# caidj0/Raytracer-2025

Hardware: NVIDIA B200
Metric: paths_per_sec (higher is better)
Workload: dtype f64

## Files before the change

raytracer-2025_b200/csrc/api.cu:

```cuda
#include <cuda_runtime.h>

#include <algorithm>
#include <cstdio>
#include <cstdlib>
#include <cstring>
#include <memory>
#include <mutex>
#include <new>
#include <string>
#include <thread>
#include <vector>

#include "compile.h"
#include "kernels.h"
#include "rt2025.h"

using namespace rt;

namespace {

thread_local std::string g_err;

int set_err(int code, const std::string& msg) {
    g_err = msg;
// ... 326 lines not shown
            v.nodes = a.put(cs.nodes, st), v.geom = a.put(cs.geom, st), v.meta = a.put(cs.meta, st), v.xforms = a.put(cs.xforms, st);
            v.materials = a.put(cs.materials, st), v.textures = a.put(cs.textures, st), v.images = a.put(cs.images, st);
            v.texels = a.put(cs.texels, st), v.perlins = a.put(cs.perlins, st), v.media = a.put(cs.media, st);
            v.lights = a.put(cs.lights, st), v.remaps = a.put(cs.remaps, st), v.walk_lean = a.put(cs.walk_lean, st);
            v.shade_lean = a.put(cs.shade_lean, st), v.shade_lean_mask = cs.shade_lean_mask;
            CU(cudaStreamSynchronize(st));
        }
        v.world_root = cs.world_root;
        v.n_media = (uint32_t)cs.media.size();
        v.n_xforms = (uint32_t)cs.xforms.size();
        v.kinds = (cs.n_spheres && !cs.n_planars) ? 1u : ((cs.n_planars && !cs.n_spheres) ? 2u : 0u);
        v.n_lights = (uint32_t)cs.lights.size();
        v.n_prims = (uint32_t)cs.geom.size();
        v.moving = 0;
        for (size_t p = 0; p < cs.geom.size(); p++)
            if ((cs.meta[p].kind_mat >> 30) == PRIM_SPHERE && (cs.geom[p].d[3] != 0.0 || cs.geom[p].d[4] != 0.0 || cs.geom[p].d[5] != 0.0)) v.moving = 1;
        s->ranks = cs.ranks;
        for (auto& m : cs.media) s->generic_media |= m.single_sphere == RT_NONE;
        v.media_xform = 0;
        for (auto& m : cs.media)
            if (m.xform != RT_NONE || (m.single_sphere != RT_NONE && cs.meta[m.single_sphere].xform != RT_NONE)) v.media_xform = 1;
        for (auto& m : cs.materials) s->class_mask |= 1u << m.shade_class;
        for (auto& t : cs.textures) s->black_texture.push_back(t.kind == RT_TEX_SOLID && t.color[0] == 0.0 && t.color[1] == 0.0 && t.color[2] == 0.0);
        uint32_t n_thick = 0, n_thick_entries = 0;
        for (auto& m : cs.media)
            if (m.flags & MEDIUM_THICK) s->class_mask |= 1u << SC_WALK, n_thick++, n_thick_entries += m.n_entry != MEDIUM_NO_ENTRIES;
        v.walk_entries_only = n_thick == 1 && n_thick_entries == 1;
        s->lights_flat = 1;
        for (auto& l : cs.lights)
            if (l.weight != 1.0 / (double)cs.lights.size()) s->lights_flat = 0;
        rt_scene_info& i = s->info;
// ... 776 lines not shown
```

raytracer-2025_b200/csrc/compile.cpp:

```cpp
#include "compile.h"

#include <omp.h>

#include <memory>
#include <parallel/algorithm>

#include <chrono>
#include <cstdio>
#include <cstdlib>

#include <vector_functions.h>

#include <algorithm>
#include <cmath>
#include <cstring>
#include <limits>

namespace rt {

namespace {

struct V3 {
    double x, y, z;
};
// ... 318 lines not shown
        double inv[9];
        if (!out_chain.inverse(inv)) return fail(RT_ERR_UNSUPPORTED, "singular Transform (zero scale)");
        return true;
    }

    bool leaf(uint32_t obj, const Affine& a, PrimGeom& g, uint32_t& kind, double lo[3], double hi[3], double* area_out, bool quiet = false) {
        const rt_object& o = d.objects[obj];
        std::memset(&g, 0, sizeof(g));
        V3 pts[8];
        int np = 0;
        double pad_r = 0.0;
        if (o.kind == RT_OBJ_SPHERE) {
            const rt_sphere& s = d.spheres[o.data];
            V3 c = v3(s.center), cv = v3(s.center_vec);
            double r = s.radius;
            g.d[0] = c.x, g.d[1] = c.y, g.d[2] = c.z, g.d[3] = cv.x, g.d[4] = cv.y, g.d[5] = cv.z, g.d[6] = r;
            kind = PRIM_SPHERE;
            if (area_out) *area_out = 0.0;
            V3 c1 = c + cv;
            bool similarity = true;
            double k = 1.0;
            if (!a.identity) {
                k = a.A[0] * a.A[0] + a.A[3] * a.A[3] + a.A[6] * a.A[6];
                for (int i = 0; i < 3 && similarity; i++)
                    for (int j = 0; j < 3; j++) {
                        double s2 = a.A[i] * a.A[j] + a.A[3 + i] * a.A[3 + j] + a.A[6 + i] * a.A[6 + j];
                        if (std::fabs(s2 - (i == j ? k : 0.0)) > 1e-9 * k) similarity = false;
                    }
            }
            if (similarity) {
                pts[np++] = a.identity ? c : a.point(c);
                pts[np++] = a.identity ? c1 : a.point(c1);
                pad_r = r * std::sqrt(k) * (1.0 + 1e-9);
            } else {
                double mn[3], mx[3];
                double cc[2][3] = {{c.x, c.y, c.z}, {c1.x, c1.y, c1.z}};
                for (int q = 0; q < 3; q++) mn[q] = std::min(cc[0][q], cc[1][q]) - r, mx[q] = std::max(cc[0][q], cc[1][q]) + r;
                for (int m = 0; m < 8; m++) pts[np++] = a.point(V3{(m & 4) ? mx[0] : mn[0], (m & 2) ? mx[1] : mn[1], (m & 1) ? mx[2] : mn[2]});
            }
        } else {
            const rt_planar& p = d.planars[o.data];
            const bool tri = o.kind == RT_OBJ_TRIANGLE;
            kind = tri ? PRIM_TRIANGLE : PRIM_QUAD;
            V3 q = v3(p.anchor), u = v3(p.u), v = v3(p.v);
            double* e = g.d;
            e[0] = q.x, e[1] = q.y, e[2] = q.z, e[3] = u.x, e[4] = u.y, e[5] = u.z, e[6] = v.x, e[7] = v.y, e[8] = v.z;
            e[9] = p.normal[0], e[10] = p.normal[1], e[11] = p.normal[2], e[12] = p.parm_d;
            e[13] = p.w[0], e[14] = p.w[1], e[15] = p.w[2];
            if (area_out) *area_out = p.area;
            V3 corner[4] = {q, q + u, q + v, q + u + v};
            for (int i = 0; i < (tri ? 3 : 4); i++) pts[np++] = a.identity ? corner[i] : a.point(corner[i]);
        }
        for (int k = 0; k < 3; k++) lo[k] = INFINITY, hi[k] = -INFINITY;
        for (int i = 0; i < np; i++) {
            double c[3] = {pts[i].x, pts[i].y, pts[i].z};
            for (int k = 0; k < 3; k++) lo[k] = std::min(lo[k], c[k] - pad_r), hi[k] = std::max(hi[k], c[k] + pad_r);
        }
        if (!a.identity) {
            for (int k = 0; k < 3; k++) {
                double m = 1e-12 * (std::fabs(lo[k]) + std::fabs(hi[k]) + (hi[k] - lo[k]));
                lo[k] -= m, hi[k] += m;
            }
        }
// ... 568 lines not shown
            med.root = roots[group_of_medium[m]];
            med.single_sphere = RT_NONE;
            if ((med.root & LEAF_FLAG) && med.root != INVALID_REF && (med.root & 7u) == 0) {
                uint32_t pi = (med.root & ~LEAF_FLAG) >> 3;
                if ((out.meta[pi].kind_mat >> 30) == PRIM_SPHERE) med.single_sphere = pi;
            }
        }
        if (timer.on) fprintf(stderr, "[rt2025 compile] %zu binary nodes (depth %u), %zu four-wide nodes (depth %u), %zu primitives\n", out.nodes.size(), out.bvh_depth, out.nodes4.size(), out.bvh4_depth, out.geom.size());
        bool all_spheres = true;
        for (const Medium& med : out.media) all_spheres = all_spheres && med.single_sphere != RT_NONE;
        double min_depth = 1.0;
        if (const char* e = getenv("RT2025_WALK_MIN_DEPTH")) min_depth = atof(e);
        for (Medium& med : out.media) {
            med.flags = 0;
            if (!all_spheres || !(min_depth > 0.0)) continue;
            const double radius = std::fabs(out.geom[med.single_sphere].d[6]);
            if (radius * std::fabs(1.0 / med.neg_inv_density) >= min_depth) med.flags |= MEDIUM_THICK;
        }
        for (size_t m = 0; m < out.media.size(); m++) {
            Medium& med = out.media[m];
            med.n_entry = MEDIUM_NO_ENTRIES;
            if (!(med.flags & MEDIUM_THICK) || getenv("RT2025_WALK_NO_ENTRIES")) continue;
            GroupBox b = group_boxes[group_of_medium[m]];
            for (int k = 0; k < 3; k++) {
                const float pad = 1e-4f * std::max(1.0f, std::max(std::fabs(b.lo[k]), std::fabs(b.hi[k])));
                b.lo[k] -= pad, b.hi[k] += pad;
            }
            uint32_t n = 0;
            const double* g = out.geom[med.single_sphere].d;
            const bool plain = med.xform == RT_NONE && out.meta[med.single_sphere].xform == RT_NONE && g[3] == 0.0 && g[4] == 0.0 && g[5] == 0.0;
            const double ball[4] = {g[0], g[1], g[2], std::fabs(g[6]) * (1.0 + 1e-4) + 1e-4};
            if (overlapping_leaves(b, plain ? ball : nullptr, out.world_root, med.entry, n)) med.n_entry = n;
            if (timer.on) fprintf(stderr, "[rt2025 compile] medium %zu is optically thick: %d entry leaves\n", m, (int)med.n_entry);
        }
        walk_lean();
        if (timer.on) fprintf(stderr, "[rt2025 compile] random walk: %s\n", out.walk_lean.empty() ? "generic" : (out.walk_lean[0].shell != RT_NONE ? "lean, shell" : "lean"));
        shade_lean();
        if (timer.on) {
            std::string classes;
            const std::pair<uint32_t, const char*> names[] = {{SC_DIFFUSE, " diffuse"}, {SC_TEXTURED, " textured"}, {SC_ISOTROPIC, " isotropic"}, {SC_EMISSIVE, " emissive"}};
            for (const auto& c : names)
                if (out.shade_lean_mask & (1u << c.first)) classes += c.second;
            fprintf(stderr, "[rt2025 compile] shade lean:%s\n", classes.empty() ? " generic" : classes.c_str());
        }
        return RT_OK;
    }
// ... 21 lines not shown
    void walk_lean() {
        out.walk_lean.clear();
        const size_t n_media = out.media.size();
        if (n_media > WALK_LEAN_MEDIA) return;
        WalkLean L;
        std::memset(&L, 0, sizeof(L));
        if (!lean_lights(L.lights)) return;
        L.n_media = (uint32_t)n_media, L.thick = RT_NONE, L.shell = RT_NONE;
        for (size_t m = 0; m < n_media; m++) {
            const Medium& med = out.media[m];
            if (med.single_sphere == RT_NONE || med.xform != RT_NONE || out.meta[med.single_sphere].xform != RT_NONE) return;
            if (med.flags & MEDIUM_THICK) {
                if (L.thick != RT_NONE || med.n_entry == MEDIUM_NO_ENTRIES) return;
                L.thick = (uint32_t)m;
            }
            std::memcpy(L.sphere[m], out.geom[med.single_sphere].d, 7 * sizeof(double));
            L.neg_inv_density[m] = med.neg_inv_density;
            L.rank[m] = med.rank, L.medium_index[m] = med.medium_index;
        }
        if (L.thick == RT_NONE) return;
        const Medium& thick = out.media[L.thick];
        if (!isotropic_axp(thick.material, L.axp)) return;
        for (uint32_t e = 0; e < thick.n_entry; e++) {
            const uint32_t first = (thick.entry[e] & ~LEAF_FLAG) >> 3, count = (thick.entry[e] & 7u) + 1;
            for (uint32_t pi = first; pi < first + count; pi++) {
                const PrimMeta& pm = out.meta[pi];
                if (L.n_prims == WALK_LEAN_PRIMS || pm.xform != RT_NONE) return;
                const uint32_t k = L.n_prims++;
                L.prim[k] = out.geom[pi];
                L.prim_kind[k] = pm.kind_mat >> 30, L.prim_rank[k] = pm.rank;
                if (L.shell == RT_NONE && L.prim_kind[k] == PRIM_SPHERE && std::memcmp(out.geom[pi].d, L.sphere[L.thick], 7 * sizeof(double)) == 0) L.shell = k;
            }
        }
        out.walk_lean.push_back(L);
    }

    void shade_lean() {
        out.shade_lean.clear();
        out.shade_lean_mask = 0;
        ShadeLean S;
        std::memset(&S, 0, sizeof(S));
        const bool lights = lean_lights(S.lights);
        bool iso = lights && out.media.size() <= SHADE_LEAN_MEDIA;
        for (size_t m = 0; iso && m < out.media.size(); m++) {
            const Medium& med = out.media[m];
            if (med.flags & MEDIUM_THICK) continue;
// ... 31 lines not shown
```

raytracer-2025_b200/csrc/kernels.cu:

```cuda
#include <cuda_runtime.h>
#include <stdint.h>

#include <algorithm>

#include "kernels.h"
#include "shade.cuh"

namespace rt {

struct RayArrayIO {
    static constexpr bool any_time = true;
    const SceneView& sv;
    const rt_ray* __restrict__ rays;
    rt_hit* __restrict__ out;
    double tmin, tmax;
    __device__ __forceinline__ double t_min() const { return tmin; }
    __device__ __forceinline__ bool load(uint32_t i, RayD& r, double& t1, uint32_t& prim0, uint32_t& rank0) const {
        const double* rp = reinterpret_cast<const double*>(rays + i);
        r.o = D3{rp[0], rp[1], rp[2]};
        r.d = D3{rp[3], rp[4], rp[5]};
        r.time = rp[6];
        t1 = tmax;
        prim0 = 0xFFFFFFFFu, rank0 = 0xFFFFFFFFu;
        return true;
// ... 1087 lines not shown
#endif

__device__ __forceinline__ bool walk_lean_segment(const SceneView& sv, const WalkLean& L, const RenderParams& P, const WavefrontState& W, const RayD& r,
                                                  D3 beta, uint32_t pixel, uint32_t sidx, uint32_t segment, double t, uint32_t max_steps,
                                                  uint32_t& steps, RayD& nr, D3& nbeta, double& tn, bool& stay) {
    stay = false;
    if (!lean_isotropic_scatter(sv, L.lights, ld3(L.axp), P, W, r, beta, pixel, sidx, segment, t, nr, nbeta)) return false;

    const uint32_t seg1 = segment + 1u, thick = L.thick;
    MediumDraws draws;
    double near_root, far_root;
    {
        const double* s = L.sphere[thick];
        double t1, t2;
        const double xi = draws.get(P.seed, pixel, sidx, seg1, L.medium_index[thick]);
        const bool inside = sphere_entry_exit_at(ld3(s), ld3(s + 3), s[6], nr, t1, t2, near_root, far_root);
        if (!inside || !medium_free_flight(t1, t2, nr, L.neg_inv_density[thick], xi, tn)) return true;
    }
    if (!(++steps < max_steps)) return true;
    const uint32_t med_rank = L.rank[thick];
    for (uint32_t m = 0; m < L.n_media; m++) {
        if (m == thick) continue;
        const double xi = draws.get(P.seed, pixel, sidx, seg1, L.medium_index[m]);
        if (RT_MEDIA_EARLY_SCREEN && free_flight_overshoots(L.neg_inv_density[m], xi, tn, nr.d)) continue;
        const double* s = L.sphere[m];
        double t1, t2, nroot, froot, tm;
        if (!sphere_entry_exit_at(ld3(s), ld3(s + 3), s[6], nr, t1, t2, nroot, froot) || !medium_free_flight(t1, t2, nr, L.neg_inv_density[m], xi, tm)) continue;
        if (tm < tn || (tm == tn && L.rank[m] < med_rank)) return true;
    }
    bool beaten = false;
    for (uint32_t i = 0; i < L.n_prims && !beaten; i++) {
        const double* g = L.prim[i].d;
        double th;
        bool hit;
        if (i == L.shell) {
            th = near_root;
            hit = contains(1e-8, tn, th);
            if (!hit) {
                th = far_root;
                hit = contains(1e-8, tn, th);
            }
        } else if (L.prim_kind[i] == PRIM_SPHERE) {
            hit = sphere_hit_at(ld3(g), ld3(g + 3), g[6], nr, 1e-8, tn, th);
        } else {
            Planar pl;
            load_planar_plain(g, pl);
            double a, b;
            hit = planar_hit_loaded(pl, L.prim_kind[i] == PRIM_TRIANGLE, nr, 1e-8, tn, th, a, b);
        }
        beaten = hit && (th < tn || L.prim_rank[i] < med_rank);
    }
    stay = !beaten;
    return true;
}

template <bool XF, bool ENTRIES, bool LEAN = false>
__global__ void __launch_bounds__(WALK_BLOCK, LEAN ? RT_WALK_LEAN_MIN_BLOCKS : RT_WALK_MIN_BLOCKS) k_walk(SceneView sv, RenderParams P, WavefrontState W) {
    extern __shared__ float4 s_mem[];
// ... 416 lines not shown
```

raytracer-2025_b200/csrc/scene_types.h:

```cpp
#pragma once
#include <stdint.h>

namespace rt {

constexpr uint32_t LEAF_FLAG = 0x80000000u;
constexpr uint32_t INVALID_REF = 0x7FFFFFFFu;
constexpr int MAX_LEAF_PRIMS = 8;
constexpr int TRAVERSAL_STACK = 64;
constexpr uint32_t META_MAT_MASK = 0x03FFFFFFu;
constexpr uint32_t META_CLASS_SHIFT = 26;

struct alignas(32) Node {
    float lo0[3], hi0[3];
    float lo1[3], hi1[3];
    uint32_t child0, child1;
    uint32_t pad0, pad1;
};
static_assert(sizeof(Node) == 64, "node must be 64 bytes");

struct alignas(32) Node4 {
    float box[4][6];
    uint32_t child[4];
    uint32_t pad[4];
};
static_assert(sizeof(Node4) == 128, "wide node must be 128 bytes");

enum PrimKind : uint32_t { PRIM_SPHERE = 0, PRIM_QUAD = 1, PRIM_TRIANGLE = 2 };

struct alignas(32) PrimGeom {
    double d[16];
};
static_assert(sizeof(PrimGeom) == 128, "primitive record must be 128 bytes");

struct alignas(16) PrimMeta {
    uint32_t kind_mat;
    uint32_t rank;
    uint32_t object;
    uint32_t xform;
};

constexpr int MAX_XFORM_CHAIN = 4;
struct Xform {
// ... 60 lines not shown
    uint32_t xform;
    double weight, cdf, area;
};

constexpr uint32_t LEAN_LIGHTS = 4;
struct LeanLights {
    Light lights[LEAN_LIGHTS];
    uint32_t n;
    uint32_t pad[7];
};

constexpr uint32_t WALK_LEAN_MEDIA = 4, WALK_LEAN_PRIMS = 8;
struct WalkLean {
    LeanLights lights;
    PrimGeom prim[WALK_LEAN_PRIMS];
    double sphere[WALK_LEAN_MEDIA][8];
    double neg_inv_density[WALK_LEAN_MEDIA];
    double axp[3];
    double pad0;
    uint32_t rank[WALK_LEAN_MEDIA], medium_index[WALK_LEAN_MEDIA];
    uint32_t prim_kind[WALK_LEAN_PRIMS], prim_rank[WALK_LEAN_PRIMS];
    uint32_t n_media, thick, n_prims;
    uint32_t shell;
};

constexpr uint32_t SHADE_LEAN_MEDIA = 4;
struct ShadeLean {
    LeanLights lights;
    double axp[SHADE_LEAN_MEDIA][4];
};

// ... 52 lines not shown
```

raytracer-2025_b200/csrc/shade.cuh:

```cuda
#pragma once
#include "disney.cuh"
#include "traverse.cuh"

namespace rt {

__device__ __forceinline__ int32_t as_i32_sat(double x) {
    if (isnan(x)) return 0;
    if (x >= 2147483647.0) return 2147483647;
    if (x <= -2147483648.0) return (-2147483647 - 1);
    return (int32_t)x;
}
__device__ __forceinline__ uint32_t as_u32_sat(double x) {
    if (!(x > 0.0)) return 0u;
    if (x >= 4294967295.0) return 0xFFFFFFFFu;
    return (uint32_t)x;
}

__device__ inline double perlin_noise(const Perlin* __restrict__ tab, D3 p) {
    double fx = floor(p.x), fy = floor(p.y), fz = floor(p.z);
    long long i = (long long)fx, j = (long long)fy, k = (long long)fz;
    double u = p.x - fx, v = p.y - fy, w = p.z - fz;
    double uu = u * u * (3.0 - 2.0 * u), vv = v * v * (3.0 - 2.0 * v), ww = w * w * (3.0 - 2.0 * w);
    double accum = 0.0;
#pragma unroll
// ... 108 lines not shown
        ok = unit_vector(qrotate(p.q, ns), h.normal) && ok;
    }
    return ok;
}

__device__ inline bool surface_hit_info(const SceneView& sv, uint32_t prim, double t, const RayD& world_ray, bool want_uv, HitInfo& h) {
    const PrimMeta m = sv.meta[prim];
    const uint32_t kind = m.kind_mat >> 30;
    h.material = m.kind_mat & META_MAT_MASK;
    const double* g = sv.geom[prim].d;
    const RayD r = m.xform == RT_NONE ? world_ray : ray_to_local(sv, m.xform, world_ray);
    D3 outward;
    h.p = r.o + t * r.d;
    h.u = 0.0, h.v = 0.0;
    if (kind == PRIM_SPHERE) {
        D3 center = ld3(g), cvec = ld3(g + 3);
        double radius = g[6];
        D3 current_center = center + r.time * cvec;
        outward = (h.p - current_center) / radius;
        if (want_uv) sphere_uv(outward, h.u, h.v);
    } else {
        Planar pl;
        load_planar(g, pl);
        outward = pl.n;
        D3 hp = h.p - pl.q;
        h.u = dot(pl.w, cross(hp, pl.v));
        h.v = dot(pl.w, cross(pl.u, hp));
    }
    h.front_face = dot(r.d, outward) < 0.0;
    h.normal = h.front_face ? outward : -outward;
    if (m.xform != RT_NONE) return hit_to_world(sv, m.xform, h);
    return true;
// ... 21 lines not shown
__device__ inline double light_leaf_pdf(const SceneView& sv, const Light& l, D3 origin, D3 direction) {
    if (!STAGED && l.xform != RT_NONE) {
        const Xform* x = sv.xforms + l.xform;
        for (uint32_t k = 0; k < x->n_chain; k++) {
            XformParams p = load_xform(sv.xforms + x->chain[k]);
            D3 lo = xf_detransform(p, origin);
            D3 lt = xf_detransform(p, origin + direction);
            origin = lo;
            direction = lt - lo;
        }
    }
    RayD r{origin, direction, 0.0};
    const double* g = l.g.d;
    if (l.kind == PRIM_SPHERE) {
        double t;
        if (!(STAGED ? sphere_hit_at(ld3(g), ld3(g + 3), g[6], r, 1e-8, INFINITY, t) : sphere_hit(g, r, 1e-8, INFINITY, t))) return 0.0;
        D3 center = ld3(g);
        double radius = g[6];
        double dist_squared = length_squared((center + 0.0 * ld3(g + 3)) - origin);
        double cos_theta_max = sqrt(1.0 - radius * radius / dist_squared);
        if (isnan(cos_theta_max)) return 1.0 / (4.0 * RT_PI);
        double solid_angle = 2.0 * RT_PI * (1.0 - cos_theta_max);
        return 1.0 / solid_angle;
    }
    Planar pl;
    if (STAGED)
        load_planar_plain(g, pl);
    else
        load_planar(g, pl);
    double t, a, b2;
    if (!planar_hit_loaded(pl, l.kind == PRIM_TRIANGLE, r, 1e-8, INFINITY, t, a, b2)) return 0.0;
    double distance_squared = t * t * length_squared(direction);
    double cosine = fabs(dot(direction, pl.n) / length(direction));
    return distance_squared / (cosine * l.area);
// ... 1 lines not shown

__device__ inline double lights_pdf_value(const SceneView& sv, uint32_t lights_flat, D3 origin, D3 direction) {
    double sum = 0.0;
    if (lights_flat) {
        for (uint32_t i = 0; i < sv.n_lights; i++) sum += light_leaf_pdf(sv, sv.lights[i], origin, direction);
        return sum / (double)sv.n_lights;
    }
    for (uint32_t i = 0; i < sv.n_lights; i++) sum += sv.lights[i].weight * light_leaf_pdf(sv, sv.lights[i], origin, direction);
    return sum;
}

__device__ inline bool light_leaf_random(const Light& l, D3 origin, double r1, double r2, D3& dir) {
    const double* g = l.g.d;
    bool ok = true;
    if (l.kind == PRIM_SPHERE) {
        D3 center = ld3(g);
        double radius = g[6];
        D3 direction = (center + 0.0 * ld3(g + 3)) - origin;
        double distance_squared = length_squared(direction);
        D3 ud;
        ok = unit_vector(direction, ud);
        ONB uvw;
        ok = make_onb(ud, uvw) && ok;
        double y = 1.0 + r2 * (sqrt(1.0 - radius * radius / distance_squared) - 1.0);
        double phi = 2.0 * RT_PI * r1;
        double s, c;
        sincos(phi, &s, &c);
        double x = c * sqrt(1.0 - y * y);
        double z = s * sqrt(1.0 - y * y);
        ok = unit_vector(onb_to_world(uvw, D3{x, y, z}), dir) && ok;
    } else {
        double ul = r1, vl = r2;
        if (l.kind == PRIM_TRIANGLE && ul + vl > 1.0) {
            double nu = 1.0 - vl, nv = 1.0 - ul;
            ul = nu, vl = nv;
        }
        D3 p = ld3(g) + (ul * ld3(g + 3)) + (vl * ld3(g + 6));
        ok = unit_vector(p - origin, dir);
    }
    return ok;
}

__device__ inline bool lights_random(const SceneView& sv, D3 origin, double pick, double r1, double r2, D3& out) {
    uint32_t leaf = sv.n_lights - 1;
    for (uint32_t i = 0; i < sv.n_lights; i++)
        if (pick < sv.lights[i].cdf) {
            leaf = i;
            break;
        }
    const Light& l = sv.lights[leaf];
    if (l.xform == RT_NONE) return light_leaf_random(l, origin, r1, r2, out);
    const Xform* x = sv.xforms + l.xform;
// ... 73 lines not shown
```

raytracer-2025_b200/csrc/traverse.cuh:

```cuda
#pragma once
#include "device_math.cuh"
#include "scene_types.h"

namespace rt {

struct RayD {
    D3 o, d;
    double time;
};

struct Quat {
    double w, x, y, z;
};
__device__ __forceinline__ Quat qmul(Quat a, Quat b) {
    return Quat{a.w * b.w - a.x * b.x - a.y * b.y - a.z * b.z, a.w * b.x + a.x * b.w + a.y * b.z - a.z * b.y,
                a.w * b.y - a.x * b.z + a.y * b.w + a.z * b.x, a.w * b.z + a.x * b.y - a.y * b.x + a.z * b.w};
}
__device__ __forceinline__ D3 qrotate(Quat q, D3 v) {
    Quat r = qmul(qmul(q, Quat{0.0, v.x, v.y, v.z}), Quat{q.w, -q.x, -q.y, -q.z});
    return D3{r.x, r.y, r.z};
}
struct XformParams {
    D3 offset, scale;
    Quat q;
// ... 117 lines not shown
    D3 oc = current_center - r.o;
    double a = length_squared(r.d);
    double h = dot(r.d, oc);
    double c = length_squared(oc) - radius * radius;
    double discriminant = h * h - a * c;
    if (discriminant < 0.0) return false;
    double sqrtd = sqrt(discriminant);
    double root = (h - sqrtd) / a;
    if (!contains(tmin, tmax, root)) {
        root = (h + sqrtd) / a;
        if (!contains(tmin, tmax, root)) return false;
    }
    t_out = root;
    return true;
}
__device__ __forceinline__ bool sphere_hit(const double* __restrict__ g, const RayD& r, double tmin, double tmax, double& t_out) {
    double2 a0, a1, a2, a3;
    ldg256(g, a0, a1);
    ldg256(g + 4, a2, a3);
    return sphere_hit_at(D3{a0.x, a0.y, a1.x}, D3{a1.y, a2.x, a2.y}, a3.x, r, tmin, tmax, t_out);
}

struct Planar {
    D3 q, u, v, n, w;
    double D;
};
__device__ __forceinline__ void load_planar(const double* __restrict__ g, Planar& p) {
    const double2* s = reinterpret_cast<const double2*>(g);
    double2 a0 = __ldg(s), a1 = __ldg(s + 1), a2 = __ldg(s + 2), a3 = __ldg(s + 3);
    double2 a4 = __ldg(s + 4), a5 = __ldg(s + 5), a6 = __ldg(s + 6), a7 = __ldg(s + 7);
    p.q = D3{a0.x, a0.y, a1.x};
    p.u = D3{a1.y, a2.x, a2.y};
    p.v = D3{a3.x, a3.y, a4.x};
    p.n = D3{a4.y, a5.x, a5.y};
    p.D = a6.x;
    p.w = D3{a6.y, a7.x, a7.y};
}
__device__ __forceinline__ void load_planar_plain(const double* g, Planar& p) {
    p.q = ld3(g), p.u = ld3(g + 3), p.v = ld3(g + 6), p.n = ld3(g + 9);
    p.D = g[12];
    p.w = ld3(g + 13);
}
__device__ __forceinline__ bool planar_hit_loaded(const Planar& p, bool triangle, const RayD& r, double tmin, double tmax,
                                                  double& t_out, double& alpha, double& beta) {
    double denom = dot(p.n, r.d);
    if (fabs(denom) < 1e-8) return false;
    double t = (p.D - dot(p.n, r.o)) / denom;
    if (!contains(tmin, tmax, t)) return false;
    D3 intersection = r.o + t * r.d;
    D3 hp = intersection - p.q;
    alpha = dot(p.w, cross(hp, p.v));
    beta = dot(p.w, cross(p.u, hp));
    if (!contains(0.0, 1.0, alpha) || !contains(0.0, 1.0, beta)) return false;
    if (triangle && !contains(0.0, 1.0, alpha + beta)) return false;
    t_out = t;
    return true;
}
__device__ __forceinline__ bool planar_hit(const double* __restrict__ g, bool triangle, const RayD& r, double tmin, double tmax, double& t_out) {
    double2 a4, a5, a6, a7;
    ldg256(g + 8, a4, a5);
    ldg256(g + 12, a6, a7);
    D3 n = D3{a4.y, a5.x, a5.y};
    double denom = dot(n, r.d);
    if (fabs(denom) < 1e-8) return false;
    double t = (a6.x - dot(n, r.o)) / denom;
    if (!contains(tmin, tmax, t)) return false;
    double2 a0, a1, a2, a3;
    ldg256(g, a0, a1);
    ldg256(g + 4, a2, a3);
    D3 q = D3{a0.x, a0.y, a1.x}, u = D3{a1.y, a2.x, a2.y}, v = D3{a3.x, a3.y, a4.x}, w = D3{a6.y, a7.x, a7.y};
    D3 intersection = r.o + t * r.d;
    D3 hp = intersection - q;
    double alpha = dot(w, cross(hp, v));
    double beta = dot(w, cross(u, hp));
    if (!contains(0.0, 1.0, alpha) || !contains(0.0, 1.0, beta)) return false;
    if (triangle && !contains(0.0, 1.0, alpha + beta)) return false;
    t_out = t;
    return true;
}

struct TraceCounters {
    uint32_t nodes, prims;
};

constexpr uint32_t SMEM_NODE_BYTES = 56;
__device__ __forceinline__ uint32_t cached_tree_float4(const SceneView& sv) {
    return sv.nodes4 ? 8u * sv.n_cached_nodes : (sv.n_cached_nodes * SMEM_NODE_BYTES + 15u) / 16u;
}
__device__ __forceinline__ void stage_nodes(const SceneView& sv, float4* smem_nodes) {
    __shared__ alignas(8) unsigned long long s_bar;
    const uint32_t bar = (uint32_t)__cvta_generic_to_shared(&s_bar);
    if (threadIdx.x == 0) {
        asm volatile("mbarrier.init.shared::cta.b64 [%0], 1;" ::"r"(bar));
// ... 39 lines not shown
            : "memory");
    }
}

template <bool COUNT, bool USE_RANK, bool ANY_TIME>
__device__ __forceinline__ bool closest_hit(const SceneView& sv, uint32_t root, const RayD& r, double tmin, double tmax,
                                            const float4* __restrict__ smem_nodes, uint32_t* __restrict__ stack, int stride,
                                            double& best_t, uint32_t& best_prim, TraceCounters* cnt) {
    if (root == INVALID_REF) return false;
    double tbest = tmax;
    uint32_t prim = 0xFFFFFFFFu, prim_rank = 0xFFFFFFFFu;
    uint32_t cached_xform = 0xFFFFFFFFu;
    RayD lr = r;
    float tmax_f = __double2float_ru(tmax);

    auto test_leaf = [&](uint32_t leaf) {
        uint32_t first = (leaf & ~LEAF_FLAG) >> 3, count = (leaf & 7u) + 1;
        for (uint32_t i = 0; i < count; i++) {
            uint32_t pi = first + i;
            const uint4 km = __ldg(reinterpret_cast<const uint4*>(&sv.meta[pi]));
            const uint32_t kind = km.x >> 30;
            if (km.w != cached_xform) {
                lr = km.w == 0xFFFFFFFFu ? r : ray_to_local(sv, km.w, r);
                cached_xform = km.w;
            }
            const double* g = sv.geom[pi].d;
            double t;
            bool hit = kind == PRIM_SPHERE ? sphere_hit(g, lr, tmin, tbest, t) : planar_hit(g, kind == PRIM_TRIANGLE, lr, tmin, tbest, t);
            if (COUNT) cnt->prims++;
            if (hit) {
                bool better = prim == 0xFFFFFFFFu || t < tbest || (USE_RANK && km.y < prim_rank);
                if (better) {
                    tbest = t;
                    prim = pi;
                    prim_rank = km.y;
                    tmax_f = __double2float_ru(t);
                }
            }
        }
    };

    if (root & LEAF_FLAG) {
        test_leaf(root);
// ... 42 lines not shown
                    cur = sp > 0 ? stack[(--sp) * stride] : INVALID_REF;
                }
            }
        }
    }
    if (prim == 0xFFFFFFFFu) return false;
    best_t = tbest;
    best_prim = prim;
    return true;
}

__device__ __forceinline__ bool leaf_beats_scatter(const SceneView& sv, uint32_t leaf, const RayD& r, double tmin, double t_scatter, uint32_t rank) {
    const uint32_t first = (leaf & ~LEAF_FLAG) >> 3, count = (leaf & 7u) + 1;
    uint32_t cached_xform = 0xFFFFFFFFu;
    RayD lr = r;
    bool beaten = false;
    for (uint32_t i = 0; i < count; i++) {
        const uint32_t pi = first + i;
        const uint4 km = __ldg(reinterpret_cast<const uint4*>(&sv.meta[pi]));
        if (km.w != cached_xform) {
            lr = km.w == 0xFFFFFFFFu ? r : ray_to_local(sv, km.w, r);
            cached_xform = km.w;
        }
        const double* g = sv.geom[pi].d;
        const uint32_t kind = km.x >> 30;
        double t;
        const bool hit = kind == PRIM_SPHERE ? sphere_hit(g, lr, tmin, t_scatter, t) : planar_hit(g, kind == PRIM_TRIANGLE, lr, tmin, t_scatter, t);
        beaten = beaten || (hit && (t < t_scatter || km.y < rank));
    }
    return beaten;
}

constexpr uint32_t FIFO_SLOT_WORDS = 28;
constexpr uint32_t FIFO_INVALID_ITEM = 0xFFFFFFFFu;

template <bool COUNT, bool USE_RANK, bool PARK, int WIDE, bool XF, int KINDS, bool ANY = false, class IO>
__device__ __forceinline__ void trace_persistent(const SceneView& sv, IO& io, uint32_t n, uint32_t* s_cursor,
                                                 const float4* __restrict__ smem_nodes, uint32_t* __restrict__ stack, int stride,
                                                 uint32_t* __restrict__ fifo, uint32_t fifo_slots_arg, TraceCounters* cnt, double* __restrict__ ray_s = nullptr) {
    const uint32_t fifo_slots = WIDE >= 2 ? 0u : fifo_slots_arg;
    constexpr bool FIFO_ONLY = WIDE == 1;
    const unsigned FULL = 0xFFFFFFFFu;
// ... 243 lines not shown
                    if ((cur & LEAF_FLAG) && parked == INVALID_REF) {
                        parked = cur;
                        cur = sp > 0 ? stack[(--sp) * stride] : INVALID_REF;
                    }
#if RT_PARK_VOTE
                    if (!__any_sync(__activemask(), parked == INVALID_REF)) break;
#endif
                } else if (cur & LEAF_FLAG) {
                    parked = cur;
                    cur = sp > 0 ? stack[(--sp) * stride] : INVALID_REF;
                    break;
                }
            }
            while (parked != INVALID_REF) {
                const uint32_t first = (parked & ~LEAF_FLAG) >> 3, count = (parked & 7u) + 1;
                for (uint32_t i = 0; i < count; i++) {
                    const uint32_t pi = first + i;
                    const uint4 km = __ldg(reinterpret_cast<const uint4*>(&sv.meta[pi]));
                    const uint32_t kind = km.x >> 30;
#if RT_RAY_SMEM
                    if (km.w != 0xFFFFFFFFu && km.w != cached_xform) {
                        put_ray(7, ray_to_local(sv, km.w, get_ray(0)));
                        cached_xform = km.w;
                    }
                    const RayD lr = get_ray(km.w == 0xFFFFFFFFu ? 0 : 7);
#else
                    if (XF && km.w != cached_xform) {
                        lr = km.w == 0xFFFFFFFFu ? r : ray_to_local(sv, km.w, r);
                        cached_xform = km.w;
                    }
#endif
                    const double* g = sv.geom[pi].d;
                    double t;
                    const RayD& tr = XF ? lr : r;
                    bool hit = KINDS == 1   ? sphere_hit(g, tr, tmin, tbest, t)
                               : KINDS == 2 ? planar_hit(g, kind == PRIM_TRIANGLE, tr, tmin, tbest, t)
                               : kind == PRIM_SPHERE ? sphere_hit(g, tr, tmin, tbest, t) : planar_hit(g, kind == PRIM_TRIANGLE, tr, tmin, tbest, t);
                    if (COUNT) cnt->prims++;
                    if (ANY) {
                        if (hit) {
                            prim = pi;
                            cur = INVALID_REF;
                            break;
                        }
                    } else if (hit && (prim == 0xFFFFFFFFu || t < tbest || (USE_RANK && km.y < prim_rank))) {
                        tbest = t;
                        prim = pi;
                        prim_rank = km.y;
                        prim_meta = km.x;
                        tmax_f = __double2float_ru(t);
                    }
                }
// ... 27 lines not shown
    if (!contains(-INFINITY, INFINITY, first)) {
        first = far_root;
        if (!contains(-INFINITY, INFINITY, first)) return false;
    }
    const double lo = first + 0.0001;
    double second = near_root;
    if (!contains(lo, INFINITY, second)) {
        second = far_root;
        if (!contains(lo, INFINITY, second)) return false;
    }
    t1 = first;
    t2 = second;
    return true;
}
__device__ __forceinline__ bool sphere_entry_exit(const double* __restrict__ g, const RayD& r, double& t1, double& t2) {
    const double2 a0 = __ldg(reinterpret_cast<const double2*>(g));
    const double2 a1 = __ldg(reinterpret_cast<const double2*>(g) + 1);
    const double2 a2 = __ldg(reinterpret_cast<const double2*>(g) + 2);
    const double2 a3 = __ldg(reinterpret_cast<const double2*>(g) + 3);
    double near_root, far_root;
    return sphere_entry_exit_at(D3{a0.x, a0.y, a1.x}, D3{a1.y, a2.x, a2.y}, a3.x, r, t1, t2, near_root, far_root);
}

__device__ __forceinline__ bool medium_free_flight(double t1, double t2, const RayD& lr, double neg_inv_density, double xi, double& tm) {
    if (t1 < 1e-8) t1 = 1e-8;
    if (t1 >= t2) return false;
    if (t1 < 0.0) t1 = 0.0;
    const double ray_length = length(lr.d);
    const double distance_inside_boundary = (t2 - t1) * ray_length;
    const float hf = (float)neg_inv_density * logf((float)xi);
    const float hf_err = 4e-7f * fabsf((float)neg_inv_density);
    if (hf > (float)distance_inside_boundary * 1.001f + hf_err) return false;
    const double hit_distance = neg_inv_density * log(xi);
    if (hit_distance > distance_inside_boundary) return false;
    tm = t1 + hit_distance / ray_length;
    return true;
// ... 11 lines not shown
```

Measured before the change: 1.584 billion.

## Reorder primitive geometry so hit-test data sits in first 64 bytes

Reorders the per-primitive geometry record so the fields needed first by a hit test come first: sphere center, radius, then motion vector, and planar normal and plane offset. A shared routine loads this 64-byte head with two 256-bit loads before the test. Planar rejection therefore needs only the head, and the rest of the record is fetched only after the plane-distance test passes. The change also adds optional leaf prefetch hooks and a common per-primitive test helper. In exchange the transformed-primitive path reloads the head after changing the ray's coordinate frame, and every consumer of the record depends on the new layout constants being used consistently.

After: 1.629 billion (median of 6 runs). 1.03x the previous value.

```diff
diff --git a/raytracer-2025_b200/csrc/api.cu b/raytracer-2025_b200/csrc/api.cu
--- a/raytracer-2025_b200/csrc/api.cu
+++ b/raytracer-2025_b200/csrc/api.cu
@@ -364,7 +364,7 @@
         v.n_prims = (uint32_t)cs.geom.size();
         v.moving = 0;
         for (size_t p = 0; p < cs.geom.size(); p++)
-            if ((cs.meta[p].kind_mat >> 30) == PRIM_SPHERE && (cs.geom[p].d[3] != 0.0 || cs.geom[p].d[4] != 0.0 || cs.geom[p].d[5] != 0.0)) v.moving = 1;
+            if ((cs.meta[p].kind_mat >> 30) == PRIM_SPHERE && (cs.geom[p].d[GEOM_SPHERE_CVEC] != 0.0 || cs.geom[p].d[GEOM_SPHERE_CVEC + 1] != 0.0 || cs.geom[p].d[GEOM_SPHERE_CVEC + 2] != 0.0)) v.moving = 1;
         s->ranks = cs.ranks;
         for (auto& m : cs.media) s->generic_media |= m.single_sphere == RT_NONE;
         v.media_xform = 0;
diff --git a/raytracer-2025_b200/csrc/compile.cpp b/raytracer-2025_b200/csrc/compile.cpp
--- a/raytracer-2025_b200/csrc/compile.cpp
+++ b/raytracer-2025_b200/csrc/compile.cpp
@@ -356,7 +356,10 @@
             const rt_sphere& s = d.spheres[o.data];
             V3 c = v3(s.center), cv = v3(s.center_vec);
             double r = s.radius;
-            g.d[0] = c.x, g.d[1] = c.y, g.d[2] = c.z, g.d[3] = cv.x, g.d[4] = cv.y, g.d[5] = cv.z, g.d[6] = r;
+            double* e = g.d;
+            e[GEOM_SPHERE_CENTER] = c.x, e[GEOM_SPHERE_CENTER + 1] = c.y, e[GEOM_SPHERE_CENTER + 2] = c.z;
+            e[GEOM_SPHERE_CVEC] = cv.x, e[GEOM_SPHERE_CVEC + 1] = cv.y, e[GEOM_SPHERE_CVEC + 2] = cv.z;
+            e[GEOM_SPHERE_RADIUS] = r;
             kind = PRIM_SPHERE;
             if (area_out) *area_out = 0.0;
             V3 c1 = c + cv;
@@ -386,9 +389,12 @@
             kind = tri ? PRIM_TRIANGLE : PRIM_QUAD;
             V3 q = v3(p.anchor), u = v3(p.u), v = v3(p.v);
             double* e = g.d;
-            e[0] = q.x, e[1] = q.y, e[2] = q.z, e[3] = u.x, e[4] = u.y, e[5] = u.z, e[6] = v.x, e[7] = v.y, e[8] = v.z;
-            e[9] = p.normal[0], e[10] = p.normal[1], e[11] = p.normal[2], e[12] = p.parm_d;
-            e[13] = p.w[0], e[14] = p.w[1], e[15] = p.w[2];
+            e[GEOM_PLANAR_Q] = q.x, e[GEOM_PLANAR_Q + 1] = q.y, e[GEOM_PLANAR_Q + 2] = q.z;
+            e[GEOM_PLANAR_U] = u.x, e[GEOM_PLANAR_U + 1] = u.y, e[GEOM_PLANAR_U + 2] = u.z;
+            e[GEOM_PLANAR_V] = v.x, e[GEOM_PLANAR_V + 1] = v.y, e[GEOM_PLANAR_V + 2] = v.z;
+            e[GEOM_PLANAR_N] = p.normal[0], e[GEOM_PLANAR_N + 1] = p.normal[1], e[GEOM_PLANAR_N + 2] = p.normal[2];
+            e[GEOM_PLANAR_D] = p.parm_d;
+            e[GEOM_PLANAR_W] = p.w[0], e[GEOM_PLANAR_W + 1] = p.w[1], e[GEOM_PLANAR_W + 2] = p.w[2];
             if (area_out) *area_out = p.area;
             V3 corner[4] = {q, q + u, q + v, q + u + v};
             for (int i = 0; i < (tri ? 3 : 4); i++) pts[np++] = a.identity ? corner[i] : a.point(corner[i]);
@@ -987,7 +993,7 @@
         for (Medium& med : out.media) {
             med.flags = 0;
             if (!all_spheres || !(min_depth > 0.0)) continue;
-            const double radius = std::fabs(out.geom[med.single_sphere].d[6]);
+            const double radius = std::fabs(out.geom[med.single_sphere].d[GEOM_SPHERE_RADIUS]);
             if (radius * std::fabs(1.0 / med.neg_inv_density) >= min_depth) med.flags |= MEDIUM_THICK;
         }
         for (size_t m = 0; m < out.media.size(); m++) {
@@ -1001,8 +1007,9 @@
             }
             uint32_t n = 0;
             const double* g = out.geom[med.single_sphere].d;
-            const bool plain = med.xform == RT_NONE && out.meta[med.single_sphere].xform == RT_NONE && g[3] == 0.0 && g[4] == 0.0 && g[5] == 0.0;
-            const double ball[4] = {g[0], g[1], g[2], std::fabs(g[6]) * (1.0 + 1e-4) + 1e-4};
+            const double *c = g + GEOM_SPHERE_CENTER, *cv = g + GEOM_SPHERE_CVEC;
+            const bool plain = med.xform == RT_NONE && out.meta[med.single_sphere].xform == RT_NONE && cv[0] == 0.0 && cv[1] == 0.0 && cv[2] == 0.0;
+            const double ball[4] = {c[0], c[1], c[2], std::fabs(g[GEOM_SPHERE_RADIUS]) * (1.0 + 1e-4) + 1e-4};
             if (overlapping_leaves(b, plain ? ball : nullptr, out.world_root, med.entry, n)) med.n_entry = n;
             if (timer.on) fprintf(stderr, "[rt2025 compile] medium %zu is optically thick: %d entry leaves\n", m, (int)med.n_entry);
         }
@@ -1054,7 +1061,7 @@
                 if (L.thick != RT_NONE || med.n_entry == MEDIUM_NO_ENTRIES) return;
                 L.thick = (uint32_t)m;
             }
-            std::memcpy(L.sphere[m], out.geom[med.single_sphere].d, 7 * sizeof(double));
+            std::memcpy(L.sphere[m], out.geom[med.single_sphere].d, GEOM_HEAD * sizeof(double));
             L.neg_inv_density[m] = med.neg_inv_density;
             L.rank[m] = med.rank, L.medium_index[m] = med.medium_index;
         }
@@ -1069,7 +1076,7 @@
                 const uint32_t k = L.n_prims++;
                 L.prim[k] = out.geom[pi];
                 L.prim_kind[k] = pm.kind_mat >> 30, L.prim_rank[k] = pm.rank;
-                if (L.shell == RT_NONE && L.prim_kind[k] == PRIM_SPHERE && std::memcmp(out.geom[pi].d, L.sphere[L.thick], 7 * sizeof(double)) == 0) L.shell = k;
+                if (L.shell == RT_NONE && L.prim_kind[k] == PRIM_SPHERE && std::memcmp(out.geom[pi].d, L.sphere[L.thick], GEOM_HEAD * sizeof(double)) == 0) L.shell = k;
             }
         }
         out.walk_lean.push_back(L);
diff --git a/raytracer-2025_b200/csrc/kernels.cu b/raytracer-2025_b200/csrc/kernels.cu
--- a/raytracer-2025_b200/csrc/kernels.cu
+++ b/raytracer-2025_b200/csrc/kernels.cu
@@ -1125,7 +1125,7 @@
         const double* s = L.sphere[thick];
         double t1, t2;
         const double xi = draws.get(P.seed, pixel, sidx, seg1, L.medium_index[thick]);
-        const bool inside = sphere_entry_exit_at(ld3(s), ld3(s + 3), s[6], nr, t1, t2, near_root, far_root);
+        const bool inside = sphere_entry_exit_at(ld3(s + GEOM_SPHERE_CENTER), ld3(s + GEOM_SPHERE_CVEC), s[GEOM_SPHERE_RADIUS], nr, t1, t2, near_root, far_root);
         if (!inside || !medium_free_flight(t1, t2, nr, L.neg_inv_density[thick], xi, tn)) return true;
     }
     if (!(++steps < max_steps)) return true;
@@ -1136,7 +1136,9 @@
         if (RT_MEDIA_EARLY_SCREEN && free_flight_overshoots(L.neg_inv_density[m], xi, tn, nr.d)) continue;
         const double* s = L.sphere[m];
         double t1, t2, nroot, froot, tm;
-        if (!sphere_entry_exit_at(ld3(s), ld3(s + 3), s[6], nr, t1, t2, nroot, froot) || !medium_free_flight(t1, t2, nr, L.neg_inv_density[m], xi, tm)) continue;
+        if (!sphere_entry_exit_at(ld3(s + GEOM_SPHERE_CENTER), ld3(s + GEOM_SPHERE_CVEC), s[GEOM_SPHERE_RADIUS], nr, t1, t2, nroot, froot) ||
+            !medium_free_flight(t1, t2, nr, L.neg_inv_density[m], xi, tm))
+            continue;
         if (tm < tn || (tm == tn && L.rank[m] < med_rank)) return true;
     }
     bool beaten = false;
@@ -1152,7 +1154,7 @@
                 hit = contains(1e-8, tn, th);
             }
         } else if (L.prim_kind[i] == PRIM_SPHERE) {
-            hit = sphere_hit_at(ld3(g), ld3(g + 3), g[6], nr, 1e-8, tn, th);
+            hit = sphere_hit_at(ld3(g + GEOM_SPHERE_CENTER), ld3(g + GEOM_SPHERE_CVEC), g[GEOM_SPHERE_RADIUS], nr, 1e-8, tn, th);
         } else {
             Planar pl;
             load_planar_plain(g, pl);
diff --git a/raytracer-2025_b200/csrc/scene_types.h b/raytracer-2025_b200/csrc/scene_types.h
--- a/raytracer-2025_b200/csrc/scene_types.h
+++ b/raytracer-2025_b200/csrc/scene_types.h
@@ -26,6 +26,10 @@
 static_assert(sizeof(Node4) == 128, "wide node must be 128 bytes");
 
 enum PrimKind : uint32_t { PRIM_SPHERE = 0, PRIM_QUAD = 1, PRIM_TRIANGLE = 2 };
+
+constexpr int GEOM_HEAD = 8;
+constexpr int GEOM_SPHERE_CENTER = 0, GEOM_SPHERE_RADIUS = 3, GEOM_SPHERE_CVEC = 4;
+constexpr int GEOM_PLANAR_N = 0, GEOM_PLANAR_D = 3, GEOM_PLANAR_Q = 4, GEOM_PLANAR_U = 7, GEOM_PLANAR_V = 10, GEOM_PLANAR_W = 13;
 
 struct alignas(32) PrimGeom {
     double d[16];
@@ -116,7 +120,7 @@
 struct WalkLean {
     LeanLights lights;
     PrimGeom prim[WALK_LEAN_PRIMS];
-    double sphere[WALK_LEAN_MEDIA][8];
+    double sphere[WALK_LEAN_MEDIA][GEOM_HEAD];
     double neg_inv_density[WALK_LEAN_MEDIA];
     double axp[3];
     double pad0;
diff --git a/raytracer-2025_b200/csrc/shade.cuh b/raytracer-2025_b200/csrc/shade.cuh
--- a/raytracer-2025_b200/csrc/shade.cuh
+++ b/raytracer-2025_b200/csrc/shade.cuh
@@ -146,8 +146,8 @@
     h.p = r.o + t * r.d;
     h.u = 0.0, h.v = 0.0;
     if (kind == PRIM_SPHERE) {
-        D3 center = ld3(g), cvec = ld3(g + 3);
-        double radius = g[6];
+        D3 center = ld3(g + GEOM_SPHERE_CENTER), cvec = ld3(g + GEOM_SPHERE_CVEC);
+        double radius = g[GEOM_SPHERE_RADIUS];
         D3 current_center = center + r.time * cvec;
         outward = (h.p - current_center) / radius;
         if (want_uv) sphere_uv(outward, h.u, h.v);
@@ -199,10 +199,12 @@
     const double* g = l.g.d;
     if (l.kind == PRIM_SPHERE) {
         double t;
-        if (!(STAGED ? sphere_hit_at(ld3(g), ld3(g + 3), g[6], r, 1e-8, INFINITY, t) : sphere_hit(g, r, 1e-8, INFINITY, t))) return 0.0;
-        D3 center = ld3(g);
-        double radius = g[6];
-        double dist_squared = length_squared((center + 0.0 * ld3(g + 3)) - origin);
+        if (!(STAGED ? sphere_hit_at(ld3(g + GEOM_SPHERE_CENTER), ld3(g + GEOM_SPHERE_CVEC), g[GEOM_SPHERE_RADIUS], r, 1e-8, INFINITY, t)
+                     : sphere_hit(g, r, 1e-8, INFINITY, t)))
+            return 0.0;
+        D3 center = ld3(g + GEOM_SPHERE_CENTER);
+        double radius = g[GEOM_SPHERE_RADIUS];
+        double dist_squared = length_squared((center + 0.0 * ld3(g + GEOM_SPHERE_CVEC)) - origin);
         double cos_theta_max = sqrt(1.0 - radius * radius / dist_squared);
         if (isnan(cos_theta_max)) return 1.0 / (4.0 * RT_PI);
         double solid_angle = 2.0 * RT_PI * (1.0 - cos_theta_max);
@@ -234,9 +236,9 @@
     const double* g = l.g.d;
     bool ok = true;
     if (l.kind == PRIM_SPHERE) {
-        D3 center = ld3(g);
-        double radius = g[6];
-        D3 direction = (center + 0.0 * ld3(g + 3)) - origin;
+        D3 center = ld3(g + GEOM_SPHERE_CENTER);
+        double radius = g[GEOM_SPHERE_RADIUS];
+        D3 direction = (center + 0.0 * ld3(g + GEOM_SPHERE_CVEC)) - origin;
         double distance_squared = length_squared(direction);
         D3 ud;
         ok = unit_vector(direction, ud);
@@ -255,7 +257,7 @@
             double nu = 1.0 - vl, nv = 1.0 - ul;
             ul = nu, vl = nv;
         }
-        D3 p = ld3(g) + (ul * ld3(g + 3)) + (vl * ld3(g + 6));
+        D3 p = ld3(g + GEOM_PLANAR_Q) + (ul * ld3(g + GEOM_PLANAR_U)) + (vl * ld3(g + GEOM_PLANAR_V));
         ok = unit_vector(p - origin, dir);
     }
     return ok;
diff --git a/raytracer-2025_b200/csrc/traverse.cuh b/raytracer-2025_b200/csrc/traverse.cuh
--- a/raytracer-2025_b200/csrc/traverse.cuh
+++ b/raytracer-2025_b200/csrc/traverse.cuh
@@ -155,32 +155,37 @@
     t_out = root;
     return true;
 }
-__device__ __forceinline__ bool sphere_hit(const double* __restrict__ g, const RayD& r, double tmin, double tmax, double& t_out) {
+__device__ __forceinline__ void ldg_head(const double* __restrict__ g, double h[GEOM_HEAD]) {
     double2 a0, a1, a2, a3;
     ldg256(g, a0, a1);
     ldg256(g + 4, a2, a3);
-    return sphere_hit_at(D3{a0.x, a0.y, a1.x}, D3{a1.y, a2.x, a2.y}, a3.x, r, tmin, tmax, t_out);
+    h[0] = a0.x, h[1] = a0.y, h[2] = a1.x, h[3] = a1.y, h[4] = a2.x, h[5] = a2.y, h[6] = a3.x, h[7] = a3.y;
+}
+__device__ __forceinline__ bool sphere_hit_head(const double* h, const RayD& r, double tmin, double tmax, double& t_out) {
+    return sphere_hit_at(ld3(h + GEOM_SPHERE_CENTER), ld3(h + GEOM_SPHERE_CVEC), h[GEOM_SPHERE_RADIUS], r, tmin, tmax, t_out);
+}
+__device__ __forceinline__ bool sphere_hit(const double* __restrict__ g, const RayD& r, double tmin, double tmax, double& t_out) {
+    double h[GEOM_HEAD];
+    ldg_head(g, h);
+    return sphere_hit_head(h, r, tmin, tmax, t_out);
 }
 
 struct Planar {
     D3 q, u, v, n, w;
     double D;
 };
+__device__ __forceinline__ void load_planar_plain(const double* g, Planar& p) {
+    p.q = ld3(g + GEOM_PLANAR_Q), p.u = ld3(g + GEOM_PLANAR_U), p.v = ld3(g + GEOM_PLANAR_V), p.n = ld3(g + GEOM_PLANAR_N);
+    p.D = g[GEOM_PLANAR_D];
+    p.w = ld3(g + GEOM_PLANAR_W);
+}
 __device__ __forceinline__ void load_planar(const double* __restrict__ g, Planar& p) {
-    const double2* s = reinterpret_cast<const double2*>(g);
-    double2 a0 = __ldg(s), a1 = __ldg(s + 1), a2 = __ldg(s + 2), a3 = __ldg(s + 3);
-    double2 a4 = __ldg(s + 4), a5 = __ldg(s + 5), a6 = __ldg(s + 6), a7 = __ldg(s + 7);
-    p.q = D3{a0.x, a0.y, a1.x};
-    p.u = D3{a1.y, a2.x, a2.y};
-    p.v = D3{a3.x, a3.y, a4.x};
-    p.n = D3{a4.y, a5.x, a5.y};
-    p.D = a6.x;
-    p.w = D3{a6.y, a7.x, a7.y};
-}
-__device__ __forceinline__ void load_planar_plain(const double* g, Planar& p) {
-    p.q = ld3(g), p.u = ld3(g + 3), p.v = ld3(g + 6), p.n = ld3(g + 9);
-    p.D = g[12];
-    p.w = ld3(g + 13);
+    double e[16];
+    for (int k = 0; k < 8; k++) {
+        const double2 a = __ldg(reinterpret_cast<const double2*>(g) + k);
+        e[2 * k] = a.x, e[2 * k + 1] = a.y;
+    }
+    load_planar_plain(e, p);
 }
 __device__ __forceinline__ bool planar_hit_loaded(const Planar& p, bool triangle, const RayD& r, double tmin, double tmax,
                                                   double& t_out, double& alpha, double& beta) {
@@ -197,19 +202,19 @@
     t_out = t;
     return true;
 }
-__device__ __forceinline__ bool planar_hit(const double* __restrict__ g, bool triangle, const RayD& r, double tmin, double tmax, double& t_out) {
-    double2 a4, a5, a6, a7;
-    ldg256(g + 8, a4, a5);
-    ldg256(g + 12, a6, a7);
-    D3 n = D3{a4.y, a5.x, a5.y};
+__device__ __forceinline__ bool planar_hit_head(const double* __restrict__ g, const double* h, bool triangle, const RayD& r, double tmin,
+                                                double tmax, double& t_out) {
+    const D3 n = ld3(h + GEOM_PLANAR_N);
     double denom = dot(n, r.d);
     if (fabs(denom) < 1e-8) return false;
-    double t = (a6.x - dot(n, r.o)) / denom;
+    double t = (h[GEOM_PLANAR_D] - dot(n, r.o)) / denom;
     if (!contains(tmin, tmax, t)) return false;
-    double2 a0, a1, a2, a3;
-    ldg256(g, a0, a1);
+    double e[16];
+    double2 a2, a3;
     ldg256(g + 4, a2, a3);
-    D3 q = D3{a0.x, a0.y, a1.x}, u = D3{a1.y, a2.x, a2.y}, v = D3{a3.x, a3.y, a4.x}, w = D3{a6.y, a7.x, a7.y};
+    e[4] = a2.x, e[5] = a2.y, e[6] = a3.x, e[7] = a3.y;
+    ldg_head(g + GEOM_HEAD, e + GEOM_HEAD);
+    D3 q = ld3(e + GEOM_PLANAR_Q), u = ld3(e + GEOM_PLANAR_U), v = ld3(e + GEOM_PLANAR_V), w = ld3(e + GEOM_PLANAR_W);
     D3 intersection = r.o + t * r.d;
     D3 hp = intersection - q;
     double alpha = dot(w, cross(hp, v));
@@ -218,6 +223,24 @@
     if (triangle && !contains(0.0, 1.0, alpha + beta)) return false;
     t_out = t;
     return true;
+}
+
+template <int KINDS, bool XF, class ToLocal, class LocalRay>
+__device__ __forceinline__ bool prim_test(const SceneView& sv, uint32_t pi, uint32_t& cached_xform, ToLocal&& to_local, LocalRay&& local_ray,
+                                          double tmin, double tmax, uint4& km, double& t_out) {
+    const double* __restrict__ g = sv.geom[pi].d;
+    km = __ldg(reinterpret_cast<const uint4*>(&sv.meta[pi]));
+    double h[GEOM_HEAD];
+    ldg_head(g, h);
+    if (XF && km.w != cached_xform) {
+        to_local(km.w);
+        cached_xform = km.w;
+        ldg_head(g, h);
+    }
+    const RayD& r = local_ray(km.w);
+    const uint32_t kind = km.x >> 30;
+    if (KINDS == 1 || (KINDS == 0 && kind == PRIM_SPHERE)) return sphere_hit_head(h, r, tmin, tmax, t_out);
+    return planar_hit_head(g, h, kind == PRIM_TRIANGLE, r, tmin, tmax, t_out);
 }
 
 struct TraceCounters {
@@ -287,19 +310,15 @@
     RayD lr = r;
     float tmax_f = __double2float_ru(tmax);
 
+    auto to_local = [&](uint32_t xform) { lr = xform == 0xFFFFFFFFu ? r : ray_to_local(sv, xform, r); };
+    auto local_ray = [&](uint32_t) -> const RayD& { return lr; };
     auto test_leaf = [&](uint32_t leaf) {
         uint32_t first = (leaf & ~LEAF_FLAG) >> 3, count = (leaf & 7u) + 1;
         for (uint32_t i = 0; i < count; i++) {
             uint32_t pi = first + i;
-            const uint4 km = __ldg(reinterpret_cast<const uint4*>(&sv.meta[pi]));
-            const uint32_t kind = km.x >> 30;
-            if (km.w != cached_xform) {
-                lr = km.w == 0xFFFFFFFFu ? r : ray_to_local(sv, km.w, r);
-                cached_xform = km.w;
-            }
-            const double* g = sv.geom[pi].d;
+            uint4 km;
             double t;
-            bool hit = kind == PRIM_SPHERE ? sphere_hit(g, lr, tmin, tbest, t) : planar_hit(g, kind == PRIM_TRIANGLE, lr, tmin, tbest, t);
+            bool hit = prim_test<0, true>(sv, pi, cached_xform, to_local, local_ray, tmin, tbest, km, t);
             if (COUNT) cnt->prims++;
             if (hit) {
                 bool better = prim == 0xFFFFFFFFu || t < tbest || (USE_RANK && km.y < prim_rank);
@@ -372,18 +391,13 @@
     const uint32_t first = (leaf & ~LEAF_FLAG) >> 3, count = (leaf & 7u) + 1;
     uint32_t cached_xform = 0xFFFFFFFFu;
     RayD lr = r;
+    auto to_local = [&](uint32_t xform) { lr = xform == 0xFFFFFFFFu ? r : ray_to_local(sv, xform, r); };
+    auto local_ray = [&](uint32_t) -> const RayD& { return lr; };
     bool beaten = false;
     for (uint32_t i = 0; i < count; i++) {
-        const uint32_t pi = first + i;
-        const uint4 km = __ldg(reinterpret_cast<const uint4*>(&sv.meta[pi]));
-        if (km.w != cached_xform) {
-            lr = km.w == 0xFFFFFFFFu ? r : ray_to_local(sv, km.w, r);
-            cached_xform = km.w;
-        }
-        const double* g = sv.geom[pi].d;
-        const uint32_t kind = km.x >> 30;
+        uint4 km;
         double t;
-        const bool hit = kind == PRIM_SPHERE ? sphere_hit(g, lr, tmin, t_scatter, t) : planar_hit(g, kind == PRIM_TRIANGLE, lr, tmin, t_scatter, t);
+        const bool hit = prim_test<0, true>(sv, first + i, cached_xform, to_local, local_ray, tmin, t_scatter, km, t);
         beaten = beaten || (hit && (t < t_scatter || km.y < rank));
     }
     return beaten;
@@ -657,28 +671,26 @@
             }
             while (parked != INVALID_REF) {
                 const uint32_t first = (parked & ~LEAF_FLAG) >> 3, count = (parked & 7u) + 1;
+#if RT_RAY_SMEM
+                auto to_local = [&](uint32_t xform) {
+                    if (xform != 0xFFFFFFFFu) put_ray(7, ray_to_local(sv, xform, get_ray(0)));
+                };
+                auto local_ray = [&](uint32_t xform) { return get_ray(xform == 0xFFFFFFFFu ? 0 : 7); };
+#else
+                auto to_local = [&](uint32_t xform) { lr = xform == 0xFFFFFFFFu ? r : ray_to_local(sv, xform, r); };
+                auto local_ray = [&](uint32_t) -> const RayD& { return XF ? lr : r; };
+#endif
+#if RT_LEAF_PREFETCH == 2
+                for (uint32_t i = 1; i < count; i++) asm volatile("prefetch.global.L1 [%0];" ::"l"(sv.geom + first + i));
+#endif
                 for (uint32_t i = 0; i < count; i++) {
                     const uint32_t pi = first + i;
-                    const uint4 km = __ldg(reinterpret_cast<const uint4*>(&sv.meta[pi]));
-                    const uint32_t kind = km.x >> 30;
-#if RT_RAY_SMEM
-                    if (km.w != 0xFFFFFFFFu && km.w != cached_xform) {
-                        put_ray(7, ray_to_local(sv, km.w, get_ray(0)));
-                        cached_xform = km.w;
-                    }
-                    const RayD lr = get_ray(km.w == 0xFFFFFFFFu ? 0 : 7);
-#else
-                    if (XF && km.w != cached_xform) {
-                        lr = km.w == 0xFFFFFFFFu ? r : ray_to_local(sv, km.w, r);
-                        cached_xform = km.w;
-                    }
-#endif
-                    const double* g = sv.geom[pi].d;
+#if RT_LEAF_PREFETCH == 1
+                    if (i + 1 < count) asm volatile("prefetch.global.L1 [%0];" ::"l"(sv.geom + pi + 1));
+#endif
+                    uint4 km;
                     double t;
-                    const RayD& tr = XF ? lr : r;
-                    bool hit = KINDS == 1   ? sphere_hit(g, tr, tmin, tbest, t)
-                               : KINDS == 2 ? planar_hit(g, kind == PRIM_TRIANGLE, tr, tmin, tbest, t)
-                               : kind == PRIM_SPHERE ? sphere_hit(g, tr, tmin, tbest, t) : planar_hit(g, kind == PRIM_TRIANGLE, tr, tmin, tbest, t);
+                    bool hit = prim_test<KINDS, XF>(sv, pi, cached_xform, to_local, local_ray, tmin, tbest, km, t);
                     if (COUNT) cnt->prims++;
                     if (ANY) {
                         if (hit) {
@@ -736,12 +748,13 @@
     return true;
 }
 __device__ __forceinline__ bool sphere_entry_exit(const double* __restrict__ g, const RayD& r, double& t1, double& t2) {
-    const double2 a0 = __ldg(reinterpret_cast<const double2*>(g));
-    const double2 a1 = __ldg(reinterpret_cast<const double2*>(g) + 1);
-    const double2 a2 = __ldg(reinterpret_cast<const double2*>(g) + 2);
-    const double2 a3 = __ldg(reinterpret_cast<const double2*>(g) + 3);
+    double h[GEOM_HEAD];
+    for (int k = 0; k < GEOM_HEAD / 2; k++) {
+        const double2 a = __ldg(reinterpret_cast<const double2*>(g) + k);
+        h[2 * k] = a.x, h[2 * k + 1] = a.y;
+    }
     double near_root, far_root;
-    return sphere_entry_exit_at(D3{a0.x, a0.y, a1.x}, D3{a1.y, a2.x, a2.y}, a3.x, r, t1, t2, near_root, far_root);
+    return sphere_entry_exit_at(ld3(h + GEOM_SPHERE_CENTER), ld3(h + GEOM_SPHERE_CVEC), h[GEOM_SPHERE_RADIUS], r, t1, t2, near_root, far_root);
 }
 
 __device__ __forceinline__ bool medium_free_flight(double t1, double t2, const RayD& lr, double neg_inv_density, double xi, double& tm) {
```
